# HPC-Research-Lab/GNN

Measured on AMD Instinct MI355X. Metric: mini-batches/sec + SpMM HBM GB/s, Reddit GraphSAGE/LADIES at 1/2/4/8 MI355X, higher is better.
Workload: dtype f32

## Files before the change

gnn_amd/csrc/step.hip:

```cpp
#include <hip/hip_runtime.h>
#include <rocblas/rocblas.h>

#include <algorithm>
#include <climits>
#include <cstdint>
#include <cstdlib>
#include <cstring>
#include <memory>
#include <mutex>
#include <string>

#include "common.h"
#include "gnn_layers.h"
#include "gnn_spmm.h"
#include "gnn_step.h"

namespace {

using gnn::align_up;
using gnn::ceil_div;

__global__ __launch_bounds__(256) void colsum_kernel(const float* __restrict__ dz, int M, int C,
                                                     float* __restrict__ out) {
  __shared__ float red[4];
  const int c = blockIdx.x;
  float s = 0.0f;
  for (int r = threadIdx.x; r < M; r += 256) s += dz[(int64_t)r * C + c];
#pragma unroll
  for (int m = 32; m >= 1; m >>= 1) s += __shfl_xor(s, m);
  if ((threadIdx.x & 63) == 0) red[threadIdx.x >> 6] = s;
  __syncthreads();
  if (threadIdx.x == 0) out[c] = (red[0] + red[1]) + (red[2] + red[3]);
}

struct Arena {
  char* base;
  size_t off = 0;
  template <typename T>
  T* take(int64_t count) {
    const size_t bytes = align_up((size_t)(count > 0 ? count : 1) * sizeof(T), 256);
    T* p = base ? (T*)(base + off) : nullptr;
    off += bytes;
    return p;
  }
};

int64_t L(const int64_t* d, int l, int f) { return d[GNN_STEP_HEADER + l * GNN_STEP_LAYER_SLOTS + f]; }
template <typename T>
T* P(const int64_t* d, int l, int f) {
  return (T*)(uintptr_t)L(d, l, f);
}
template <typename T>
T* HP(const int64_t* d, int f) {
  return (T*)(uintptr_t)d[f];
}

bool fills(int64_t M, int64_t N, int n) { return ceil_div(M, 128) * ceil_div(N, 128) * n >= 256; }
bool gemm_ok(const void* p, int64_t ld) { return ((uintptr_t)p % 8) == 0 && (ld % 2) == 0; }

std::mutex g_blas_mu;
rocblas_handle g_blas[64][2] = {};

int blas_handle(rocblas_handle* h, int which = 0) {
  int dev = 0;
  GNN_HIP(hipGetDevice(&dev), "hipGetDevice");
  GNN_REQUIRE(dev >= 0 && dev < 64, "gnn_train_step: device index %d", dev);
  std::lock_guard<std::mutex> g(g_blas_mu);
  if (!g_blas[dev][which]) {
    if (rocblas_create_handle(&g_blas[dev][which]) != rocblas_status_success)
      return gnn::fail(-1, "rocblas_create_handle failed");
  }
  *h = g_blas[dev][which];
  return 0;
}

struct Aux {
  hipStream_t s = nullptr;
  hipEvent_t ev[24] = {};
  int next = 0;
  std::mutex mu;
  hipEvent_t take() { return ev[next++ % 24]; }
};
std::mutex g_aux_mu;
Aux* g_aux[64][4] = {};

int aux_of(hipStream_t st, Aux** out) {
  int dev = 0;
  GNN_HIP(hipGetDevice(&dev), "hipGetDevice");
  GNN_REQUIRE(dev >= 0 && dev < 64, "gnn_train_step: device index %d", dev);
  int prio = 0, lo = 0, hi = 0;
  GNN_HIP(hipStreamGetPriority(st, &prio), "hipStreamGetPriority");
  GNN_HIP(hipDeviceGetStreamPriorityRange(&lo, &hi), "hipDeviceGetStreamPriorityRange");
  const int slot = std::min(3, std::max(0, lo - prio));
  std::lock_guard<std::mutex> g(g_aux_mu);
  Aux*& a = g_aux[dev][slot];
  if (!a) {
    std::unique_ptr<Aux> n(new Aux());
    GNN_HIP(hipStreamCreateWithPriority(&n->s, hipStreamNonBlocking, prio), "hipStreamCreateWithPriority");
    for (auto& e : n->ev) GNN_HIP(hipEventCreateWithFlags(&e, hipEventDisableTiming), "hipEventCreateWithFlags");
    a = n.release();
  }
  *out = a;
  return 0;
}

int fork_join(Aux* a, hipStream_t from, hipStream_t to) {
  hipEvent_t e = a->take();
  GNN_HIP(hipEventRecord(e, from), "hipEventRecord");
  GNN_HIP(hipStreamWaitEvent(to, e, 0), "hipStreamWaitEvent");
  return 0;
}

bool no_index() {
  const char* e = getenv("GNN_STEP_GATHER");
  const char* a = getenv("GNN_GEMM_ALGO");
  return (e && atoi(e) != 0) || (a && std::string(a) == "f32");
}

bool f32_gemm() {
  const char* e = getenv("GNN_GEMM_ALGO");
  return e && std::string(e) == "f32";
}

int gemm(int ak, int bk, int64_t M, int64_t N, int64_t K, int nb, const float* const* A, int64_t lda,
         const float* const* B, int64_t ldb, float* const* C, int64_t ldc, void* ws, size_t wsb, hipStream_t st) {
  if (f32_gemm()) return gnn_gemm_f32(ak, bk, M, N, K, nb, A, lda, B, ldb, C, ldc, ws, wsb, st);
  return gnn_gemm_f32_split3(ak, bk, M, N, K, nb, A, lda, B, ldb, C, ldc, ws, wsb, st);
}

size_t gemm_ws(int64_t M, int64_t N, int64_t K, int nb) {
  return std::max(gnn_gemm_f32_split3_workspace_bytes(M, N, K, nb), gnn_gemm_f32_workspace_bytes(M, N, K, nb));
}

bool fuse_agg_enabled() {
  const char* e = getenv("GNN_STEP_FUSE_AGG");
  return !(e && atoi(e) == 0);
}

bool small_overlap_enabled() {
  const char* e = getenv("GNN_STEP_SMALL_OVERLAP");
  return !(e && atoi(e) == 0);
}

bool overlap_enabled() {
  const char* e = getenv("GNN_STEP_OVERLAP");
  return e && atoi(e) != 0;
}

int sgemm(rocblas_handle h, rocblas_operation ta, rocblas_operation tb, int64_t m, int64_t n, int64_t k,
          const float* A, int64_t lda, const float* B, int64_t ldb, float* C, int64_t ldc) {
  const float one = 1.0f, zero = 0.0f;
  if (rocblas_sgemm(h, ta, tb, (rocblas_int)m, (rocblas_int)n, (rocblas_int)k, &one, A, (rocblas_int)lda, B,
                    (rocblas_int)ldb, &zero, C, (rocblas_int)ldc) != rocblas_status_success)
    return gnn::fail(-1, "rocblas_sgemm failed (m %lld n %lld k %lld)", (long long)m, (long long)n, (long long)k);
  return 0;
// ... 111 lines not shown
      b.b_gemm_dx = b.b_bwd = 0;
    }
  }
  for (int l = 0; l < pl.nl - 1; ++l) pl.lb[l].dY = ar.take<float>(pl.lb[l].M * pl.lb[l].D);
  return 0;
}

#define GNN_TRY(x)        \
  do {                    \
    int rc_ = (x);        \
    if (rc_) return rc_;  \
  } while (0)

}

extern "C" {

size_t gnn_train_step_workspace_bytes(const int64_t* desc) {
  if (!desc) return 0;
  Arena ar{nullptr};
  Plan pl;
  if (plan(desc, ar, pl)) return 0;
  return ar.off;
}

int gnn_train_step_f32(const int64_t* d, void* workspace, size_t workspace_bytes, void* stream) {
  GNN_REQUIRE(d != nullptr, "gnn_train_step: NULL descriptor");
  Arena ar{(char*)workspace};
  Plan pl;
  {
    Arena dry{nullptr};
    Plan tmp;
    GNN_TRY(plan(d, dry, tmp));
    GNN_REQUIRE(workspace && workspace_bytes >= dry.off, "gnn_train_step: workspace too small (%zu < %zu)",
                workspace_bytes, dry.off);
    GNN_REQUIRE((uintptr_t)workspace % 256 == 0, "gnn_train_step: workspace not 256-byte aligned");
  }
  GNN_TRY(plan(d, ar, pl));
  hipStream_t st = (hipStream_t)stream;
  rocblas_handle h = nullptr;
  GNN_TRY(blas_handle(&h));
  if (rocblas_set_stream(h, st) != rocblas_status_success) return gnn::fail(-1, "rocblas_set_stream failed");
  const int n = pl.sage ? 2 : 1;
  const float p = [&] {
    float f;
    const int32_t bits = (int32_t)d[GNN_SH_PDROP_BITS];
    std::memcpy(&f, &bits, 4);
    return f;
  }();
  const int training = (int)d[GNN_SH_TRAINING];
  Aux* aux = nullptr;
  const bool big_ov = overlap_enabled() && !f32_gemm();
  const bool small_ov = small_overlap_enabled();
  if (big_ov || small_ov) GNN_TRY(aux_of(st, &aux));
  std::unique_lock<std::mutex> aux_lock;
  if (aux) aux_lock = std::unique_lock<std::mutex>(aux->mu);
  bool aux_used = false;
  rocblas_handle ha = nullptr;
  if (aux && small_ov) {
    GNN_TRY(blas_handle(&ha, 1));
    if (rocblas_set_stream(ha, aux->s) != rocblas_status_success) return gnn::fail(-1, "rocblas_set_stream failed");
  }
  int64_t* const T = HP<int64_t>(d, GNN_SH_TIMING);
  int64_t nrec = 0;
  auto arm = [&](int64_t kind, int64_t l, int64_t M, int64_t K, int64_t nnz, int64_t F, int64_t Fk, int64_t ldx,
                 int64_t ldo, const void* X, const void* Y, int64_t res_rows) {
    if (!T || nrec >= T[0]) return;
    int64_t* r = T + 1 + GNN_STEP_TIMING_SLOTS * nrec++;
    gnn_spmm_set_timing_events((void*)r[0], (void*)r[1]);
    const int64_t v[] = {kind, l, M, K, nnz, F, Fk, ldx, ldo, (int64_t)(uintptr_t)X, (int64_t)(uintptr_t)Y, res_rows, 1};
    std::memcpy(r + 2, v, sizeof v);
  };
  auto stage_gate = [&](int l) -> int {
    if (d[GNN_SH_STAGE_EVENT] && l == (int)d[GNN_SH_STAGE_LAYER])
      GNN_HIP(hipEventRecord((hipEvent_t)d[GNN_SH_STAGE_EVENT], st), "hipEventRecord (stage gate)");
    return 0;
  };
  const int64_t phase = d[GNN_SH_PHASE];
  GNN_REQUIRE(phase >= 0 && phase <= 2, "gnn_train_step: phase %lld", (long long)phase);
  auto first_agg = [&]() -> int {
    const LayerBufs& b = pl.lb[0];
    return gnn_spmm_csr_f32(P<const int32_t>(d, 0, GNN_SL_ROWPTR), P<const int32_t>(d, 0, GNN_SL_COL),
                            P<const float>(d, 0, GNN_SL_VAL), b.M, b.K, b.nnz, b.X, b.ldx, b.feat, b.ldo, b.Fk,
                            b.ws_fwd, b.b_fwd, 0, st);
  };
  if (phase == 1) {
    GNN_TRY(first_agg());
    return stage_gate(0);
  }
  for (int l = 0; l < pl.nl; ++l) {
    LayerBufs& b = pl.lb[l];
    const int64_t N = b.N;
    const float* WB = P<const float>(d, l, GNN_SL_WB);
    const float* WW = P<const float>(d, l, GNN_SL_WW);
    if (pl.sage)
      GNN_REQUIRE(L(d, l, GNN_SL_NSAMPLED) == b.M, "gnn_train_step: layer %d sampled %lld != M %lld", l,
                  (long long)L(d, l, GNN_SL_NSAMPLED), (long long)b.M);
    const bool ok = gemm_ok(b.feat, b.ldo) && gemm_ok(WW, b.F) && (!pl.sage || gemm_ok(WB, b.F));
    const bool small_side = ha && pl.sage && !(ok && fills(b.M, N, n));
    if (big_ov && pl.sage && ok && fills(b.M, N, n)) {
      b.xs_gathered = true;
      GNN_TRY(fork_join(aux, st, aux->s));
      GNN_TRY(gnn_gather_rows_f32(b.X, b.ldx, P<const int64_t>(d, l, GNN_SL_SAMPLED), b.xs, b.ldo, nullptr, b.M, b.F,
                                  aux->s));
      const float* Ab[1] = {b.xs};
      const float* Bb[1] = {WB};
      float* Cb[1] = {b.hB};
      GNN_TRY(gnn::gemm_split3_as_batch(0, 0, b.M, N, b.F, 1, 2, 0, Ab, b.ldo, Bb, b.F, Cb, N, b.ws_gemm_f2, b.b_gemm_f,
                                        aux->s));
      if (phase != 2 || l != 0) {
        arm(0, l, b.M, b.K, b.nnz, b.F, b.Fk, b.ldx, b.ldo, b.X, b.feat, 0);
        GNN_TRY(gnn_spmm_csr_f32(P<const int32_t>(d, l, GNN_SL_ROWPTR), P<const int32_t>(d, l, GNN_SL_COL),
                                 P<const float>(d, l, GNN_SL_VAL), b.M, b.K, b.nnz, b.X, b.ldx, b.feat, b.ldo, b.Fk,
                                 b.ws_fwd, b.b_fwd, 0, st));
        GNN_TRY(stage_gate(l));
      }
      const float* Aw[1] = {b.feat};
      const float* Bw[1] = {WW};
      float* Cw[1] = {b.hW};
      GNN_TRY(gnn::gemm_split3_as_batch(0, 0, b.M, N, b.F, 1, 2, 1, Aw, b.ldo, Bw, b.F, Cw, N, b.ws_gemm_f, b.b_gemm_f, st));
      GNN_TRY(fork_join(aux, aux->s, st));
    } else if (small_side) {
      b.xs_gathered = true;
      GNN_TRY(fork_join(aux, st, aux->s));
      GNN_TRY(gnn_gather_rows_f32(b.X, b.ldx, P<const int64_t>(d, l, GNN_SL_SAMPLED), b.xs, b.ldo, nullptr, b.M,
                                  b.F, aux->s));
      GNN_TRY(mm_xwt(ha, b.xs, b.ldo, WB, b.F, b.hB, N, b.M, N, b.F));
      if (phase != 2 || l != 0) {
        arm(0, l, b.M, b.K, b.nnz, b.F, b.Fk, b.ldx, b.ldo, b.X, b.feat, 0);
        GNN_TRY(gnn_spmm_csr_f32(P<const int32_t>(d, l, GNN_SL_ROWPTR), P<const int32_t>(d, l, GNN_SL_COL),
                                 P<const float>(d, l, GNN_SL_VAL), b.M, b.K, b.nnz, b.X, b.ldx, b.feat, b.ldo, b.Fk,
                                 b.ws_fwd, b.b_fwd, 0, st));
        GNN_TRY(stage_gate(l));
      }
      GNN_TRY(mm_xwt(h, b.feat, b.ldo, WW, b.F, b.hW, N, b.M, N, b.F));
      GNN_TRY(fork_join(aux, aux->s, st));
    } else {
      if (phase != 2 || l != 0) {
        arm(0, l, b.M, b.K, b.nnz, b.F, b.Fk, b.ldx, b.ldo, b.X, b.feat, 0);
        GNN_TRY(gnn_spmm_csr_f32(P<const int32_t>(d, l, GNN_SL_ROWPTR), P<const int32_t>(d, l, GNN_SL_COL),
                                 P<const float>(d, l, GNN_SL_VAL), b.M, b.K, b.nnz, b.X, b.ldx, b.feat, b.ldo, b.Fk,
                                 b.ws_fwd, b.b_fwd, 0, st));
        GNN_TRY(stage_gate(l));
      }
      b.xs_gathered = !(pl.sage && ok && fills(b.M, N, n) && b.M >= 2048 && b.ldx == b.ldo && !no_index());
      if (pl.sage && b.xs_gathered)
        GNN_TRY(gnn_gather_rows_f32(b.X, b.ldx, P<const int64_t>(d, l, GNN_SL_SAMPLED), b.xs, b.ldo, nullptr, b.M,
                                    b.F, st));
    }
    if ((big_ov && pl.sage && ok && fills(b.M, N, n)) || small_side) {
    } else if (ok && fills(b.M, N, n) && !b.xs_gathered) {
      const float* A[2] = {b.X, b.feat};
      const int64_t* IA[2] = {P<const int64_t>(d, l, GNN_SL_SAMPLED), nullptr};
      const float* B[2] = {WB, WW};
      float* Cc[2] = {b.hB, b.hW};
      GNN_TRY(gnn::gemm_split3_indexed(0, 0, b.M, N, b.F, n, A, b.ldo, IA, b.K, B, b.F, nullptr, 0, Cc, N,
                                       b.ws_gemm_f, b.b_gemm_f, st));
    } else if (ok && fills(b.M, N, n)) {
      const float* A[2] = {pl.sage ? b.xs : b.feat, b.feat};
      const float* B[2] = {pl.sage ? WB : WW, WW};
      float* Cc[2] = {pl.sage ? b.hB : b.hW, b.hW};
      GNN_TRY(gemm(0, 0, b.M, N, b.F, n, A + (pl.sage ? 0 : 1), b.ldo, B + (pl.sage ? 0 : 1), b.F,
                                  Cc + (pl.sage ? 0 : 1), N, b.ws_gemm_f, b.b_gemm_f, st));
    } else {
      if (pl.sage) GNN_TRY(mm_xwt(h, b.xs, b.ldo, WB, b.F, b.hB, N, b.M, N, b.F));
      GNN_TRY(mm_xwt(h, b.feat, b.ldo, WW, b.F, b.hW, N, b.M, N, b.F));
    }
    GNN_TRY(gnn_sage_norm_fwd_f32(pl.sage ? b.hB : nullptr, pl.sage ? N : 4, pl.sage ? N : 0, b.hW, N, N,
                                  pl.sage ? P<const float>(d, l, GNN_SL_BB) : nullptr, P<const float>(d, l, GNN_SL_BW),
                                  P<const float>(d, l, GNN_SL_SCALE), P<const float>(d, l, GNN_SL_OFFSET), b.M, p,
                                  (uint64_t)L(d, l, GNN_SL_SEED), training, b.Y, b.D, b.mean, b.rstd, st));
  }
  const LayerBufs& top = pl.lb[pl.nl - 1];
  const float* Wh = HP<const float>(d, GNN_SH_HEAD_W);
  const uint64_t hseed = (uint64_t)d[GNN_SH_HEAD_SEED];
  const float* labels = HP<const float>(d, GNN_SH_LABELS);
  const int64_t ldl = d[GNN_SH_LDL];
  GNN_TRY(gnn_head_bce_fwd_f32(top.Y, top.D, pl.Mh, pl.Dh, Wh, HP<const float>(d, GNN_SH_HEAD_B), pl.C, labels, ldl, p,
                               hseed, training, pl.xd, pl.z, pl.nrm, pl.rowloss, HP<float>(d, GNN_SH_LOSS), st));
  GNN_TRY(gnn_head_bce_bwd_f32(top.Y, top.D, pl.Mh, pl.Dh, Wh, pl.C, labels, ldl, nullptr, p, hseed, training, pl.z,
                               pl.nrm, pl.dz, pl.dXh, pl.Dh, st));
  const int64_t* const E = HP<const int64_t>(d, GNN_SH_GRAD_EVENTS);
  auto grads_ready = [&](int64_t slot, hipStream_t s) -> int {
    if (E && slot < E[0] && E[slot]) GNN_HIP(hipEventRecord((hipEvent_t)E[slot], s), "hipEventRecord (grad event)");
    return 0;
  };
  bool head_pending = true;
  auto head_grads = [&](hipStream_t s, rocblas_handle hh) -> int {
    GNN_TRY(mm_gtx(hh, pl.dz, pl.C, pl.xd, pl.Dh, HP<float>(d, GNN_SH_HEAD_GW), pl.Dh, pl.C, pl.Dh, pl.Mh));
    if (HP<float>(d, GNN_SH_HEAD_GB)) {
// ... 116 lines not shown
```

gnn_amd/executor.py:

```python
from __future__ import annotations

import os
import struct
from typing import List, Optional

import numpy as np
import torch

from . import _lib
from . import custom_sparse_ops as cso

VERSION, MAX_LAYERS, HEADER, LAYER_SLOTS, SAGE, GCN = 1, 4, 24, 32, 0, 1
(H_VERSION, H_LAYERS, H_KIND, H_X0, H_LDX0, H_F0, H_HEAD_W, H_HEAD_B, H_HEAD_GW, H_HEAD_GB, H_CLASSES, H_LABELS,
 H_LDL, H_HEAD_SEED, H_PDROP_BITS, H_TRAINING, H_LOSS, H_NHID, H_TIMING, H_GRAD_EVENTS, H_STAGE_EVENT,
 H_STAGE_LAYER, H_PHASE) = range(23)
TIMING_SLOTS = 16
(L_ROWPTR, L_COL, L_VAL, L_M, L_K, L_NNZ, L_TROWPTR, L_TCOL, L_TVAL, L_SAMPLED, L_NSAMPLED, L_RMAP, L_WW, L_BW,
 L_WB, L_BB, L_SCALE, L_OFFSET, L_GWW, L_GBW, L_GWB, L_GBB, L_GSCALE, L_GOFFSET, L_SEED) = range(25)


def _p(t: Optional[torch.Tensor]) -> int:
    return 0 if t is None else t.data_ptr()


def enabled() -> bool:
    return os.environ.get("GNN_NATIVE_STEP", "1") != "0"


class NativeStep:

    def __init__(self, model):
        from . import models

        enc = model.encoder
        if not getattr(enc, "fused", False):
            raise ValueError("NativeStep needs the fused model (build_model(..., fused=True))")
        if isinstance(enc, models.GraphSage):
            self.kind = SAGE
        elif isinstance(enc, models.GCN):
            self.kind = GCN
        else:
            raise ValueError(f"NativeStep: unsupported encoder {type(enc).__name__}")
        if any(g.order != 1 for g in enc.gcs) or not 1 <= len(enc.gcs) <= MAX_LAYERS:
            raise ValueError("NativeStep: every layer must have order 1 (1-4 layers)")
        self.model = model
        self.enc = enc
        self.params: List[torch.nn.Parameter] = [p for p in model.parameters()]
        dev = self.params[0].device
        self.device = dev
        n = sum(p.numel() for p in self.params)
        self.flat_grad = torch.zeros(n, dtype=torch.float32, device=dev)
        self.grads, off = [], 0
        for p in self.params:
            self.grads.append(self.flat_grad[off:off + p.numel()].view_as(p))
            off += p.numel()
        g = {id(p): gr for p, gr in zip(self.params, self.grads)}
        d = np.zeros(HEADER + LAYER_SLOTS * len(enc.gcs), dtype=np.int64)
        d[H_VERSION] = VERSION
        d[H_LAYERS] = len(enc.gcs)
        d[H_KIND] = self.kind
        head = model.linear
        d[H_HEAD_W], d[H_HEAD_B] = _p(head.weight), _p(head.bias)
        d[H_HEAD_GW], d[H_HEAD_GB] = _p(g[id(head.weight)]), _p(g.get(id(head.bias)) if head.bias is not None else None)
        d[H_CLASSES] = head.weight.shape[0]
        d[H_NHID] = enc.gcs[0].n_out
        self.p_enc = float(enc.dropout.p)
        self.p_head = float(model.dropout.p)
        if self.p_enc != self.p_head:
# ... 10 lines not shown
            d[b + L_WW], d[b + L_BW] = _p(W.weight), _p(W.bias)
            d[b + L_GWW], d[b + L_GBW] = _p(g[id(W.weight)]), _p(g[id(W.bias)])
            d[b + L_SCALE], d[b + L_OFFSET] = _p(gc.scale), _p(gc.offset)
            d[b + L_GSCALE], d[b + L_GOFFSET] = _p(g[id(gc.scale)]), _p(g[id(gc.offset)])
        for p in self.params:
            if not (p.is_cuda and p.dtype == torch.float32 and p.is_contiguous()):
                raise ValueError("NativeStep: parameters must be contiguous float32 CUDA tensors")
        self.template = d

    def supports(self, x0, adjs, sampled_nodes, labels) -> bool:
        from .custom_sparse_ops import CsrOperand

        if not (x0.is_cuda and x0.dtype == torch.float32 and x0.stride(1) == 1 and labels.dtype == torch.float32
                and labels.dim() == 2 and labels.stride(1) == 1):
            return False
        C, D = self.model.linear.weight.shape
        if C > 256 or D % 4 or D > 2048 or labels.shape[1] != C:
            return False
        for li, op in enumerate(adjs):
            if not isinstance(op, CsrOperand):
                return False
            if li >= 1 and op._t is None:
                return False
            if self.kind == SAGE:
                s = sampled_nodes[li]
                if s.dtype != torch.int64 or not s.is_contiguous() or s.numel() != op.shape[0]:
                    return False
                if li >= 1 and getattr(s, "_gnn_rmap", None) is None:
                    return False
        return True

    def grad_stages(self):
        head = {id(p) for p in self.model.linear.parameters()}
        stages = [[i for i, p in enumerate(self.params) if id(p) in head]]
        for gc in reversed(self.enc.gcs):
            mine = {id(p) for p in gc.parameters()}
            stages.append([i for i, p in enumerate(self.params) if id(p) in mine])
        return stages

    @staticmethod
    def _batch_key(x0, adjs, labels):
        return (x0.data_ptr(), tuple(x0.shape), x0.stride(0), labels.data_ptr(), tuple(id(op) for op in adjs))

    def prefetch(self, x0, adjs, sampled_nodes, labels, stage_gate=None) -> None:
        d = self._desc(x0, adjs, sampled_nodes, labels, seeds=False)
        if stage_gate is not None and int(stage_gate[1]) == 0:
            self._set_gate(d, stage_gate)
        d[H_PHASE] = 1
        ws, wsb = self._workspace(d, x0.device)
        L = _lib.lib()
        with _lib.on_device(x0.device):
            _lib.check(L.gnn_train_step_f32(d.ctypes.data, ws.data_ptr(), wsb, _lib.stream_of(x0.device)),
                       "gnn_train_step_f32 (phase 1)")
        self._pre = (self._batch_key(x0, adjs, labels), ws, wsb, (x0, tuple(adjs), labels))

    def drop_prefetch(self) -> None:
        self._pre = None

    @staticmethod
    def _set_gate(d, stage_gate):
        ev, layer = stage_gate
        if not getattr(ev, "_gnn_created", False):
            ev.record()
            ev._gnn_created = True
        d[H_STAGE_EVENT], d[H_STAGE_LAYER] = ev.cuda_event, int(layer)

    @staticmethod
    def _workspace(d, device):
        wsb = _lib.lib().gnn_train_step_workspace_bytes(d.ctypes.data)
        if wsb == 0:
            raise RuntimeError("gnn_train_step_workspace_bytes: " + _lib.lib().gnn_last_error().decode(errors="replace"))
        return torch.empty(wsb, dtype=torch.uint8, device=device), wsb

    def step(self, x0, adjs, sampled_nodes, labels, grad_events=None, stage_gate=None) -> torch.Tensor:
        d = self._desc(x0, adjs, sampled_nodes, labels, seeds=True)
        pre, self._pre = getattr(self, "_pre", None), None
        if pre is not None and pre[0] == self._batch_key(x0, adjs, labels):
            d[H_PHASE] = 2
            ws, wsb = pre[1], pre[2]
            if stage_gate is not None and int(stage_gate[1]) == 0:
                stage_gate = None
        else:
            ws, wsb = None, 0
        loss = torch.empty((), dtype=torch.float32, device=x0.device)
        d[H_LOSS] = loss.data_ptr()
        timing = self._arm_timing(d, len(adjs)) if cso.timing_enabled() else None
        E = None
        if grad_events is not None:
            E = np.zeros(1 + len(grad_events), dtype=np.int64)
            E[0] = len(E)
            for i, ev in enumerate(grad_events):
                if ev is not None:
                    ev.record()
                    E[1 + i] = ev.cuda_event
            d[H_GRAD_EVENTS] = E.ctypes.data
        if stage_gate is not None:
            self._set_gate(d, stage_gate)
        L = _lib.lib()
        dp = d.ctypes.data
        if ws is None:
            ws, wsb = self._workspace(d, x0.device)
        with _lib.on_device(x0.device):
            _lib.check(L.gnn_train_step_f32(dp, ws.data_ptr(), wsb, _lib.stream_of(x0.device)), "gnn_train_step_f32")
        if timing is not None:
            self._collect_timing(*timing)
        for p, gr in zip(self.params, self.grads):
            p.grad = gr
        return loss

    def _desc(self, x0, adjs, sampled_nodes, labels, seeds: bool):
        model = self.model
        training = model.training
        tr = bool(training and self.p_enc > 0)
        d = self.template.copy()
        d[H_X0], d[H_LDX0], d[H_F0] = x0.data_ptr(), x0.stride(0) if x0.shape[0] > 1 else x0.shape[1], x0.shape[1]
        d[H_LABELS], d[H_LDL] = labels.data_ptr(), labels.stride(0) if labels.shape[0] > 1 else labels.shape[1]
        d[H_TRAINING] = int(tr)
        sv = torch.randint(0, 2**62, (len(adjs) + 1,)).tolist() if (tr and seeds) else None
        for li, op in enumerate(adjs):
            b = HEADER + li * LAYER_SLOTS
            d[b + L_ROWPTR], d[b + L_COL], d[b + L_VAL] = op.rowptr.data_ptr(), op.col.data_ptr(), op.val.data_ptr()
            d[b + L_M], d[b + L_K], d[b + L_NNZ] = op.shape[0], op.shape[1], op.nnz
            if li >= 1:
                t = op._t
                d[b + L_TROWPTR], d[b + L_TCOL], d[b + L_TVAL] = t.rowptr.data_ptr(), t.col.data_ptr(), t.val.data_ptr()
            if self.kind == SAGE:
                s = sampled_nodes[li]
                d[b + L_SAMPLED], d[b + L_NSAMPLED] = s.data_ptr(), s.numel()
                r = getattr(s, "_gnn_rmap", None)
                d[b + L_RMAP] = _p(r) if li >= 1 else 0
            d[b + L_SEED] = sv[li] if sv is not None else 0
        d[H_HEAD_SEED] = sv[len(adjs)] if sv is not None else 0
        return d

    @staticmethod
    def _arm_timing(d, nl):
        n = 2 * nl - 1
        T = np.zeros(1 + TIMING_SLOTS * n, dtype=np.int64)
        T[0] = n
        evs = []
        for i in range(n):
            e0, e1 = torch.cuda.Event(enable_timing=True), torch.cuda.Event(enable_timing=True)
            e0.record()
            e1.record()
            T[1 + TIMING_SLOTS * i], T[2 + TIMING_SLOTS * i] = e0.cuda_event, e1.cuda_event
            evs.append((e0, e1))
        d[H_TIMING] = T.ctypes.data
        return T, evs

    @staticmethod
    def _collect_timing(T, evs):
        for i, (e0, e1) in enumerate(evs):
            r = T[1 + TIMING_SLOTS * i: 1 + TIMING_SLOTS * (i + 1)]
            if r[14] != 1:
                continue
            kind, l, M, K, nnz, F, Fk, ldx, ldy, xp, yp, res = (int(v) for v in r[2:14])
# ... 3 lines not shown
```

gnn_amd/staging.py:

```python
from __future__ import annotations

import contextlib
import ctypes
import os
import sys
import weakref
from dataclasses import dataclass
from typing import List, Optional

import numpy as np
import torch

from . import custom_sparse_ops as cso


_WAIT_SLEEP_S = max(0.0, float(os.environ.get("GNN_WAIT_SLEEP_US", "20")) * 1e-6)
_slack_set = set()


def wait_event(ev) -> None:
    if _WAIT_SLEEP_S <= 0.0:
        ev.synchronize()
        return
    if ev.query():
# ... 68 lines not shown


@dataclass
class StagePlan:
    n_input: int
    own_pos: np.ndarray
    own_src: np.ndarray
    host_pos: np.ndarray
    host_rows: Optional[torch.Tensor]
    peer_pos: List[np.ndarray]
    peer_src: List[np.ndarray]
    pinned: tuple = ()
    blob: object = None
    peer_meta: object = None


def make_plan(host_batch, store: FeatureStore, rank: int, world_size: int, devices=None) -> StagePlan:
    devices = list(range(world_size)) if devices is None else list(devices)
    masks = host_batch.input_nodes_mask_on_devices
    idxs = host_batch.nodes_idx_on_devices
    own_pos = np.flatnonzero(masks[rank]).astype(np.int64)
    own_src = np.asarray(idxs[rank], dtype=np.int64)
    host_pos = np.flatnonzero(host_batch.input_nodes_mask_on_cpu).astype(np.int64)
    host_src = np.ascontiguousarray(host_batch.nodes_idx_on_cpu, dtype=np.int64)
    host_rows = None if store.zero_copy else store.host_rows_pinned(host_src)
    peer_pos, peer_src = [], []
    for j in range(world_size):
        if j == rank:
            peer_pos.append(np.zeros(0, np.int64))
            peer_src.append(np.zeros(0, np.int64))
        else:
            peer_pos.append(np.flatnonzero(masks[j]).astype(np.int64))
            peer_src.append(np.asarray(idxs[j], dtype=np.int64))
    cuda = torch.cuda.is_available()
    arrs = (own_pos, own_src, host_pos) + ((host_src,) if store.zero_copy else ())
    pin = tuple(torch.from_numpy(a).pin_memory() if cuda else torch.from_numpy(a) for a in arrs)
    return StagePlan(host_batch.num_input_nodes, own_pos, own_src, host_pos, host_rows, peer_pos, peer_src, pin)


def _staging_stream(device):
    cus = int(os.environ.get("GNN_STAGE_CUS", "0"))
    if cus <= 0:
        return torch.cuda.Stream(device=device)
    import ctypes

    from . import _lib

    ptr = ctypes.c_void_p()
    idx = torch.device(device).index or 0
    _lib.check(_lib.lib().gnn_stream_create_cu_masked(idx, cus, 0, ctypes.byref(ptr)), "gnn_stream_create_cu_masked")
    return torch.cuda.ExternalStream(ptr.value, device=device)


class Stager:

    def __init__(self, store: FeatureStore, exchange: Optional["PeerExchange"] = None):
        self.store = store
        self.device = store.device
        self.stream = _staging_stream(self.device)
        self.exchange = exchange
        self.timing: Optional[list] = None
        self.gate: Optional[torch.cuda.Event] = None

    def take_timing(self):
        recs, self.timing = self.timing or [], None
        if not recs:
            return 0, 0.0
        recs[-1][1].synchronize()
        return sum(b for _, _, b in recs), sum(a.elapsed_time(b) for a, b, _ in recs) * 1e-3

    def issue(self, plan: StagePlan, batch_fn=None):
        dev = self.device
        st = self.stream
        meta = None
        if self.exchange is not None:
            fut = plan.peer_meta
            if fut is not None:
                plan.peer_meta = None
                meta = fut.result()
            else:
                meta = self.exchange.prepare(plan)
        with torch.cuda.stream(st):
            x0 = torch.empty((plan.n_input, self.store.ld), dtype=torch.float32, device=dev)
            if _NATIVE_STAGE and plan.blob is not None and self.timing is None and not self.store.zero_copy:
                from .loader import ToDevice

                if isinstance(batch_fn, ToDevice) and batch_fn.host is plan.blob:
                    batch = plan.blob.stage(dev, x0, self.store, self.gate)
                    if batch_fn.on_built is not None:
                        batch_fn.on_built(batch)
                    extra = self.exchange.exchange(plan, x0, self.store, meta) if self.exchange is not None else ()
                    ev = torch.cuda.Event()
                    ev.record(st)
                    return StagedX0(x0, ev, tuple(extra) + tuple(batch.tensors()), self.store.F, batch)
            nh = len(plan.host_pos)
            if self.timing is not None:
                e0, e1 = torch.cuda.Event(enable_timing=True), torch.cuda.Event(enable_timing=True)
                e0.record(st)
            if plan.blob is not None:
                own_pos, own_src, host_pos, host_dev = plan.blob.stage_views(dev)
                if self.store.zero_copy:
                    cso.gather_rows_host(self.store.host, host_dev, x0, host_pos, n=nh)
            else:
                idx = [t.to(dev, non_blocking=True) for t in plan.pinned]
                own_pos, own_src, host_pos = idx[:3]
                if plan.host_rows is None:
                    host_dev = idx[3]
                    cso.gather_rows_host(self.store.host, host_dev, x0, host_pos, n=nh)
                else:
                    host_dev = plan.host_rows.to(dev, non_blocking=True)
            if self.timing is not None:
                e1.record(st)
                self.timing.append((e0, e1, plan.blob.nbytes if plan.blob is not None else nh * self.store.ld * 4))
            if self.gate is not None:
                st.wait_event(self.gate)
            host_rows_here = nh and (plan.host_rows is not None or (plan.blob is not None and not self.store.zero_copy))
            if host_rows_here and _GATHER2:
                cso.gather_rows2(self.store.gpu_buffer, own_src, own_pos, len(plan.own_pos), host_dev, None, host_pos,
                                 nh, x0)
            else:
                cso.gather_rows(self.store.gpu_buffer, own_src, x0, own_pos, n=len(plan.own_pos))
                if host_rows_here:
                    cso.gather_rows(host_dev, None, x0, host_pos, n=nh)
            extra = ()
            if self.exchange is not None:
                extra = self.exchange.exchange(plan, x0, self.store, meta)
            batch = batch_fn() if batch_fn is not None else None
            ev = torch.cuda.Event()
            ev.record(st)
        keep = (own_pos, own_src, host_pos, host_dev) + tuple(extra)
        if batch is not None:
            keep += tuple(batch.tensors())
        return StagedX0(x0, ev, keep, self.store.F, batch)


_EXTRACT_CHECK = os.environ.get("GNN_EXTRACT_CHECK", "step")
_GATHER2 = os.environ.get("GNN_GATHER2", "1") != "0"
_NATIVE_STAGE = os.environ.get("GNN_NATIVE_STAGE", "1") != "0" and _GATHER2


class StagedX0:
    def __init__(self, x0, event, keep, F, batch=None):
        self._x0 = x0
        self.event = event
        self._keep = keep
        self.F = F
        self.batch = batch
        self.adjs = list(batch.adjs) if batch is not None and batch.adjs is not None else None
        self.err_host = getattr(batch, "err_host", None) if batch is not None else None

    def wait(self, retire: Optional["Retirement"] = None) -> torch.Tensor:
        b = self.batch
        if b is not None and self.err_host is not None and _EXTRACT_CHECK == "step":
            wait_event(self.event)
            b.check_extraction(self.err_host)
        cur = torch.cuda.current_stream(self._x0.device)
        cur.wait_event(self.event)
        if retire is None:
            self._x0.record_stream(cur)
            for t in self._keep:
                t.record_stream(cur)
        return self._x0[:, : self.F]


class Retirement:

    def __init__(self, depth: int = 3):
        import collections

        self.depth = depth
        self.q = collections.deque()
        self.wait_s = 0.0

    def retire(self, staged) -> None:
        ev = torch.cuda.Event()
        ev.record()
        self.q.append((ev, staged))
        while self.q and self.q[0][0].query():
            self.q.popleft()
        if len(self.q) > self.depth:
            import time

            t0 = time.perf_counter()
            while len(self.q) > self.depth:
                ev0, _ = self.q.popleft()
                wait_event(ev0)
            self.wait_s += time.perf_counter() - t0

    def drain(self) -> None:
        while self.q:
            ev0, _ = self.q.popleft()
            ev0.synchronize()


class NegotiatedStream:

    def __init__(self, it, exchange: "PeerExchange", depth: int = 4):
        import collections
        from concurrent.futures import ThreadPoolExecutor

        self.it = iter(it)
        self.exchange = exchange
        self.depth = max(0, int(depth))
        self.q = collections.deque()
# ... 217 lines not shown
```

gnn_amd/train.py:

```python
from __future__ import annotations

import os
from typing import Optional

import torch
from torch._utils import _flatten_dense_tensors, _unflatten_dense_tensors

from .models import loss as loss_fn


class Trainer:
    def __init__(self, model: torch.nn.Module, lr: float, device, group=None, sigmoid_loss: bool = True,
                 clip: float = 5.0):
        self.model = model
        self.device = torch.device(device)
        self.sigmoid_loss = sigmoid_loss
        self.clip = clip
        self.group = group
        self.params = [p for p in model.parameters() if p.requires_grad]
        self.native = self.device.type == "cuda"
        if self.native:
            torch.backends.cuda.preferred_blas_library("cublas")
            from .optim import ClipAdam

# ... 26 lines not shown
        self.exchange = self.bucketed if os.environ.get("GNN_DP_BUCKETS", "0") == "1" else None
        self.stage_gate = None

    @property
    def num_params(self) -> int:
        return sum(p.numel() for p in self.params)

    def broadcast_parameters(self):
        flat = _flatten_dense_tensors([p.detach() for p in self.params])
        torch.distributed.broadcast(flat, src=0, group=self.group)
        with torch.no_grad():
            for p, v in zip(self.params, _unflatten_dense_tensors(flat, self.params)):
                p.copy_(v)

    def param_digest(self) -> str:
        import hashlib

        h = hashlib.sha256()
        for p in self.params:
            h.update(p.detach().contiguous().cpu().numpy().tobytes())
        return h.hexdigest()[:16]

    def check_ranks_agree(self) -> dict:
        d = self.param_digest()
        dist = torch.distributed
        if not (dist.is_available() and dist.is_initialized()):
            return {"identical": True, "digests": [d]}
        digests = [None] * dist.get_world_size(self.group)
        torch.distributed.all_gather_object(digests, d, group=self.group)
        return {"identical": all(x == digests[0] for x in digests), "digests": digests}

    def allreduce_grads(self) -> Optional[torch.Tensor]:
        if not self.dp:
            return None
        grads = [p.grad for p in self.params]
        flat = _flatten_dense_tensors(grads)
        torch.distributed.all_reduce(flat, op=torch.distributed.ReduceOp.SUM, group=self.group)
        for p, g in zip(self.params, _unflatten_dense_tensors(flat, grads)):
            p.grad = g
        return flat

    def _next_batch(self, prefetch):
        if prefetch is None or self.executor is None or os.environ.get("GNN_PREFETCH_L0", "1") == "0":
            return None
        from . import custom_sparse_ops as cso

        if cso.timing_enabled():
            return None
        nxt = prefetch() if callable(prefetch) else prefetch
        if nxt is None or not self.executor.supports(*nxt):
            return None
        return nxt

    def step(self, x0, adjs, sampled_nodes, labels, prefetch=None) -> torch.Tensor:
        if not self.model.training:
            self.model.train()
        if self.executor is not None and self.executor.supports(x0, adjs, sampled_nodes, labels):
            if self.exchange is not None:
                loss = self.executor.step(x0, adjs, sampled_nodes, labels, grad_events=self.exchange.events,
                                          stage_gate=self.stage_gate)
                self.exchange.issue()
                self.exchange.finish()
                self.optimizer.step(clipped=True)
                return loss
            loss = self.executor.step(x0, adjs, sampled_nodes, labels,
                                      stage_gate=self.stage_gate)
            if self.dp:
                flat = self.optimizer.clip_to_flat()
                work = torch.distributed.all_reduce(flat, op=torch.distributed.ReduceOp.SUM, group=self.group,
                                                    async_op=True)
                nxt = self._next_batch(prefetch)
                if nxt is not None:
                    self.executor.prefetch(*nxt, stage_gate=self.stage_gate)
                work.wait()
                self.optimizer.step(clipped=True)
            else:
                self.optimizer.step()
            return loss
        for p in self.params:
            p.grad = None
        if hasattr(self.model, "forward_loss"):
            loss, _ = self.model.forward_loss(x0, adjs, sampled_nodes, labels, self.sigmoid_loss)
        else:
            out = self.model(x0, adjs, sampled_nodes)
            loss = loss_fn(out, labels, self.sigmoid_loss, self.device)
        if self.native:
            one = getattr(self, "_one", None)
            if one is None or one.device != loss.device:
                one = self._one = torch.ones((), dtype=loss.dtype, device=loss.device)
            loss.backward(one)
        else:
            loss.backward()
        if self.native:
            if self.dp:
                flat = self.optimizer.clip_to_flat()
                torch.distributed.all_reduce(flat, op=torch.distributed.ReduceOp.SUM, group=self.group)
                self.optimizer.step(clipped=True)
            else:
                self.optimizer.step()
            return loss.detach()
        torch.nn.utils.clip_grad_norm_(self.params, self.clip)
        self.allreduce_grads()
        self.optimizer.step()
        return loss.detach()


DEFAULT_TIMEOUT_S = 180.0


def collective_timeout():
    import datetime

    s = float(os.environ.get("GNN_DIST_TIMEOUT_S", DEFAULT_TIMEOUT_S))
    if not s > 0:
        raise ValueError(f"GNN_DIST_TIMEOUT_S must be > 0, got {s}")
    return datetime.timedelta(seconds=s)


def init_group(backend: str, rank: Optional[int] = None, world: Optional[int] = None, local: int = 0):
# ... 34 lines not shown
```

include/gnn_step.h:

```cpp
#ifndef GNN_STEP_H
#define GNN_STEP_H

#include <stddef.h>
#include <stdint.h>

#ifdef __cplusplus
extern "C" {
#endif

#define GNN_STEP_VERSION 1
#define GNN_STEP_MAX_LAYERS 4
#define GNN_STEP_HEADER 24
#define GNN_STEP_LAYER_SLOTS 32
#define GNN_STEP_SAGE 0
#define GNN_STEP_GCN 1
#define GNN_STEP_TIMING_SLOTS 16

enum {
  GNN_SH_VERSION = 0, GNN_SH_LAYERS = 1, GNN_SH_KIND = 2, GNN_SH_X0 = 3, GNN_SH_LDX0 = 4, GNN_SH_F0 = 5,
  GNN_SH_HEAD_W = 6, GNN_SH_HEAD_B = 7, GNN_SH_HEAD_GW = 8, GNN_SH_HEAD_GB = 9, GNN_SH_CLASSES = 10,
  GNN_SH_LABELS = 11, GNN_SH_LDL = 12, GNN_SH_HEAD_SEED = 13, GNN_SH_PDROP_BITS = 14, GNN_SH_TRAINING = 15,
  GNN_SH_LOSS = 16, GNN_SH_NHID = 17, GNN_SH_TIMING = 18, GNN_SH_GRAD_EVENTS = 19, GNN_SH_STAGE_EVENT = 20,
  GNN_SH_STAGE_LAYER = 21, GNN_SH_PHASE = 22
};
enum {
  GNN_SL_ROWPTR = 0, GNN_SL_COL = 1, GNN_SL_VAL = 2, GNN_SL_M = 3, GNN_SL_K = 4, GNN_SL_NNZ = 5,
  GNN_SL_TROWPTR = 6, GNN_SL_TCOL = 7, GNN_SL_TVAL = 8, GNN_SL_SAMPLED = 9, GNN_SL_NSAMPLED = 10,
  GNN_SL_RMAP = 11, GNN_SL_WW = 12, GNN_SL_BW = 13, GNN_SL_WB = 14, GNN_SL_BB = 15, GNN_SL_SCALE = 16,
  GNN_SL_OFFSET = 17, GNN_SL_GWW = 18, GNN_SL_GBW = 19, GNN_SL_GWB = 20, GNN_SL_GBB = 21, GNN_SL_GSCALE = 22,
  GNN_SL_GOFFSET = 23, GNN_SL_SEED = 24
};

size_t gnn_train_step_workspace_bytes(const int64_t* desc);
int gnn_train_step_f32(const int64_t* desc, void* workspace, size_t workspace_bytes, void* stream);

#ifdef __cplusplus
}
#endif

#endif
```

Baseline: 608.0.

## Overlap next batch's first-layer SpMM with current step on a prefetch stream

Inside a training step, the first-layer aggregation SpMM of the next staged mini-batch is now issued on a separate low-priority prefetch stream, forked when the current step reaches its last layer. The goal is to hide that SpMM behind the tail and backward pass of the current step. A staging FIFO exposes the next staged batch, and the executor keeps the prefetched workspace and a done event so the next step can skip phase 1. This brings cross-step event plumbing, an extra workspace allocation per step, and contention for HBM bandwidth between the two streams. It is turned off for data-parallel runs, when timing is enabled, and when the stage gate sits at layer 0.

```diff
diff --git a/gnn_amd/csrc/step.hip b/gnn_amd/csrc/step.hip
--- a/gnn_amd/csrc/step.hip
+++ b/gnn_amd/csrc/step.hip
@@ -76,6 +76,7 @@
 
 struct Aux {
   hipStream_t s = nullptr;
+  hipStream_t pf = nullptr;
   hipEvent_t ev[24] = {};
   int next = 0;
   std::mutex mu;
@@ -101,6 +102,16 @@
     a = n.release();
   }
   *out = a;
+  return 0;
+}
+
+int prefetch_stream(Aux* a, hipStream_t* out) {
+  if (!a->pf) {
+    int lo = 0, hi = 0;
+    GNN_HIP(hipDeviceGetStreamPriorityRange(&lo, &hi), "hipDeviceGetStreamPriorityRange");
+    GNN_HIP(hipStreamCreateWithPriority(&a->pf, hipStreamNonBlocking, lo), "hipStreamCreateWithPriority");
+  }
+  *out = a->pf;
   return 0;
 }
 
@@ -318,7 +329,8 @@
   Aux* aux = nullptr;
   const bool big_ov = overlap_enabled() && !f32_gemm();
   const bool small_ov = small_overlap_enabled();
-  if (big_ov || small_ov) GNN_TRY(aux_of(st, &aux));
+  const int64_t* const NX = HP<const int64_t>(d, GNN_SH_NEXT);
+  if (big_ov || small_ov || NX) GNN_TRY(aux_of(st, &aux));
   std::unique_lock<std::mutex> aux_lock;
   if (aux) aux_lock = std::unique_lock<std::mutex>(aux->mu);
   bool aux_used = false;
@@ -344,14 +356,52 @@
   };
   const int64_t phase = d[GNN_SH_PHASE];
   GNN_REQUIRE(phase >= 0 && phase <= 2, "gnn_train_step: phase %lld", (long long)phase);
-  auto first_agg = [&]() -> int {
-    const LayerBufs& b = pl.lb[0];
-    return gnn_spmm_csr_f32(P<const int32_t>(d, 0, GNN_SL_ROWPTR), P<const int32_t>(d, 0, GNN_SL_COL),
-                            P<const float>(d, 0, GNN_SL_VAL), b.M, b.K, b.nnz, b.X, b.ldx, b.feat, b.ldo, b.Fk,
-                            b.ws_fwd, b.b_fwd, 0, st);
+  auto first_agg = [](const int64_t* dd, const Plan& pp, hipStream_t s) -> int {
+    const LayerBufs& b = pp.lb[0];
+    return gnn_spmm_csr_f32(P<const int32_t>(dd, 0, GNN_SL_ROWPTR), P<const int32_t>(dd, 0, GNN_SL_COL),
+                            P<const float>(dd, 0, GNN_SL_VAL), b.M, b.K, b.nnz, b.X, b.ldx, b.feat, b.ldo, b.Fk,
+                            b.ws_fwd, b.b_fwd, 0, s);
+  };
+  const int64_t* nd = nullptr;
+  Plan npl;
+  hipStream_t ps = nullptr;
+  if (NX) {
+    GNN_REQUIRE(phase != 1, "gnn_train_step: a next batch with phase 1");
+    GNN_REQUIRE(!(d[GNN_SH_STAGE_EVENT] && d[GNN_SH_STAGE_LAYER] == 0),
+                "gnn_train_step: a next batch with the staging gate at layer 0");
+    nd = HP<const int64_t>(NX, GNN_SN_DESC);
+    void* const nws = HP<void>(NX, GNN_SN_WORKSPACE);
+    const size_t nwsb = (size_t)NX[GNN_SN_WORKSPACE_BYTES];
+    GNN_REQUIRE(nd != nullptr && NX[GNN_SN_DONE] != 0, "gnn_train_step: next batch without descriptor or done event");
+    GNN_REQUIRE(nd[GNN_SH_NEXT] == 0 && nd[GNN_SH_TIMING] == 0, "gnn_train_step: next batch's descriptor is not plain");
+    Arena dry{nullptr};
+    Plan tmp;
+    GNN_TRY(plan(nd, dry, tmp));
+    GNN_REQUIRE(nws && nwsb >= dry.off, "gnn_train_step: next batch's workspace too small (%zu < %zu)", nwsb, dry.off);
+    GNN_REQUIRE((uintptr_t)nws % 256 == 0, "gnn_train_step: next batch's workspace not 256-byte aligned");
+    Arena nar{(char*)nws};
+    GNN_TRY(plan(nd, nar, npl));
+    ps = (hipStream_t)NX[GNN_SN_STREAM];
+    if (!ps) GNN_TRY(prefetch_stream(aux, &ps));
+  }
+  auto issue_next = [&](hipEvent_t e) -> int {
+    GNN_HIP(hipStreamWaitEvent(ps, e, 0), "hipStreamWaitEvent (prefetch fork)");
+    if (NX[GNN_SN_READY])
+      GNN_HIP(hipStreamWaitEvent(ps, (hipEvent_t)NX[GNN_SN_READY], 0), "hipStreamWaitEvent (prefetch ready)");
+    GNN_TRY(first_agg(nd, npl, ps));
+    GNN_HIP(hipEventRecord((hipEvent_t)NX[GNN_SN_DONE], ps), "hipEventRecord (prefetch done)");
+    return 0;
+  };
+  auto fork_fwd = [&](int l, bool to_aux) -> int {
+    if (!to_aux && !(NX && l == pl.nl - 1)) return 0;
+    hipEvent_t e = aux->take();
+    GNN_HIP(hipEventRecord(e, st), "hipEventRecord");
+    if (to_aux) GNN_HIP(hipStreamWaitEvent(aux->s, e, 0), "hipStreamWaitEvent");
+    if (NX && l == pl.nl - 1) GNN_TRY(issue_next(e));
+    return 0;
   };
   if (phase == 1) {
-    GNN_TRY(first_agg());
+    GNN_TRY(first_agg(d, pl, st));
     return stage_gate(0);
   }
   for (int l = 0; l < pl.nl; ++l) {
@@ -366,7 +416,7 @@
     const bool small_side = ha && pl.sage && !(ok && fills(b.M, N, n));
     if (big_ov && pl.sage && ok && fills(b.M, N, n)) {
       b.xs_gathered = true;
-      GNN_TRY(fork_join(aux, st, aux->s));
+      GNN_TRY(fork_fwd(l, true));
       GNN_TRY(gnn_gather_rows_f32(b.X, b.ldx, P<const int64_t>(d, l, GNN_SL_SAMPLED), b.xs, b.ldo, nullptr, b.M, b.F,
                                   aux->s));
       const float* Ab[1] = {b.xs};
@@ -388,7 +438,7 @@
       GNN_TRY(fork_join(aux, aux->s, st));
     } else if (small_side) {
       b.xs_gathered = true;
-      GNN_TRY(fork_join(aux, st, aux->s));
+      GNN_TRY(fork_fwd(l, true));
       GNN_TRY(gnn_gather_rows_f32(b.X, b.ldx, P<const int64_t>(d, l, GNN_SL_SAMPLED), b.xs, b.ldo, nullptr, b.M,
                                   b.F, aux->s));
       GNN_TRY(mm_xwt(ha, b.xs, b.ldo, WB, b.F, b.hB, N, b.M, N, b.F));
@@ -402,6 +452,7 @@
       GNN_TRY(mm_xwt(h, b.feat, b.ldo, WW, b.F, b.hW, N, b.M, N, b.F));
       GNN_TRY(fork_join(aux, aux->s, st));
     } else {
+      GNN_TRY(fork_fwd(l, false));
       if (phase != 2 || l != 0) {
         arm(0, l, b.M, b.K, b.nnz, b.F, b.Fk, b.ldx, b.ldo, b.X, b.feat, 0);
         GNN_TRY(gnn_spmm_csr_f32(P<const int32_t>(d, l, GNN_SL_ROWPTR), P<const int32_t>(d, l, GNN_SL_COL),
diff --git a/gnn_amd/executor.py b/gnn_amd/executor.py
--- a/gnn_amd/executor.py
+++ b/gnn_amd/executor.py
@@ -13,7 +13,8 @@
 VERSION, MAX_LAYERS, HEADER, LAYER_SLOTS, SAGE, GCN = 1, 4, 24, 32, 0, 1
 (H_VERSION, H_LAYERS, H_KIND, H_X0, H_LDX0, H_F0, H_HEAD_W, H_HEAD_B, H_HEAD_GW, H_HEAD_GB, H_CLASSES, H_LABELS,
  H_LDL, H_HEAD_SEED, H_PDROP_BITS, H_TRAINING, H_LOSS, H_NHID, H_TIMING, H_GRAD_EVENTS, H_STAGE_EVENT,
- H_STAGE_LAYER, H_PHASE) = range(23)
+ H_STAGE_LAYER, H_PHASE, H_NEXT) = range(24)
+(N_DESC, N_WORKSPACE, N_WORKSPACE_BYTES, N_READY, N_DONE, N_STREAM) = range(6)
 TIMING_SLOTS = 16
 (L_ROWPTR, L_COL, L_VAL, L_M, L_K, L_NNZ, L_TROWPTR, L_TCOL, L_TVAL, L_SAMPLED, L_NSAMPLED, L_RMAP, L_WW, L_BW,
  L_WB, L_BB, L_SCALE, L_OFFSET, L_GWW, L_GBW, L_GWB, L_GBB, L_GSCALE, L_GOFFSET, L_SEED) = range(25)
@@ -130,10 +131,36 @@
         with _lib.on_device(x0.device):
             _lib.check(L.gnn_train_step_f32(d.ctypes.data, ws.data_ptr(), wsb, _lib.stream_of(x0.device)),
                        "gnn_train_step_f32 (phase 1)")
-        self._pre = (self._batch_key(x0, adjs, labels), ws, wsb, (x0, tuple(adjs), labels))
+        self._release(getattr(self, "_pre", None))
+        self._pre = (self._batch_key(x0, adjs, labels), ws, wsb, (x0, tuple(adjs), labels), None, ())
 
     def drop_prefetch(self) -> None:
-        self._pre = None
+        pre, self._pre = getattr(self, "_pre", None), None
+        self._release(pre)
+
+    @staticmethod
+    def _release(pre) -> None:
+        if pre is None or pre[4] is None:
+            return
+        for st in pre[5]:
+            if st is not None:
+                st.wait_event(pre[4])
+
+    def __del__(self):
+        try:
+            self.drop_prefetch()
+        except Exception:
+            pass
+
+    def _done_event(self):
+        ring = getattr(self, "_done_ring", None)
+        if ring is None:
+            ring = self._done_ring = [torch.cuda.Event() for _ in range(4)]
+            for ev in ring:
+                ev.record()
+            self._done_i = 0
+        self._done_i = (self._done_i + 1) % len(ring)
+        return ring[self._done_i]
 
     @staticmethod
     def _set_gate(d, stage_gate):
@@ -150,16 +177,23 @@
             raise RuntimeError("gnn_train_step_workspace_bytes: " + _lib.lib().gnn_last_error().decode(errors="replace"))
         return torch.empty(wsb, dtype=torch.uint8, device=device), wsb
 
-    def step(self, x0, adjs, sampled_nodes, labels, grad_events=None, stage_gate=None) -> torch.Tensor:
+    def step(self, x0, adjs, sampled_nodes, labels, grad_events=None, stage_gate=None, next=None) -> torch.Tensor:
         d = self._desc(x0, adjs, sampled_nodes, labels, seeds=True)
         pre, self._pre = getattr(self, "_pre", None), None
+        cur = torch.cuda.current_stream(x0.device)
         if pre is not None and pre[0] == self._batch_key(x0, adjs, labels):
             d[H_PHASE] = 2
             ws, wsb = pre[1], pre[2]
+            if pre[4] is not None:
+                cur.wait_event(pre[4])
             if stage_gate is not None and int(stage_gate[1]) == 0:
                 stage_gate = None
         else:
+            self._release(pre)
             ws, wsb = None, 0
+        del pre
+        if next is not None and (cso.timing_enabled() or (stage_gate is not None and int(stage_gate[1]) == 0)):
+            next = None
         loss = torch.empty((), dtype=torch.float32, device=x0.device)
         d[H_LOSS] = loss.data_ptr()
         timing = self._arm_timing(d, len(adjs)) if cso.timing_enabled() else None
@@ -178,8 +212,24 @@
         dp = d.ctypes.data
         if ws is None:
             ws, wsb = self._workspace(d, x0.device)
+        pending = None
+        if next is not None:
+            (nx0, nadjs, nsampled, nlabels), ready, nstream = next
+            on_staging = nstream is not None and os.environ.get("GNN_PREFETCH_STREAM", "staging") != "own"
+            dn = self._desc(nx0, nadjs, nsampled, nlabels, seeds=False)
+            nws, nwsb = self._workspace(dn, x0.device)
+            done = self._done_event()
+            R = np.zeros(6, dtype=np.int64)
+            R[N_DESC], R[N_WORKSPACE], R[N_WORKSPACE_BYTES] = dn.ctypes.data, nws.data_ptr(), nwsb
+            R[N_READY] = ready.cuda_event if ready is not None else 0
+            R[N_DONE] = done.cuda_event
+            R[N_STREAM] = nstream.cuda_stream if on_staging else 0
+            d[H_NEXT] = R.ctypes.data
+            pending = (self._batch_key(nx0, nadjs, nlabels), nws, nwsb, (nx0, tuple(nadjs), nlabels), done,
+                       (cur, nstream))
         with _lib.on_device(x0.device):
             _lib.check(L.gnn_train_step_f32(dp, ws.data_ptr(), wsb, _lib.stream_of(x0.device)), "gnn_train_step_f32")
+        self._pre = pending
         if timing is not None:
             self._collect_timing(*timing)
         for p, gr in zip(self.params, self.grads):
diff --git a/gnn_amd/staging.py b/gnn_amd/staging.py
--- a/gnn_amd/staging.py
+++ b/gnn_amd/staging.py
@@ -144,6 +144,48 @@
     return torch.cuda.ExternalStream(ptr.value, device=device)
 
 
+class StageFifo:
+
+    def __init__(self):
+        self._q = {}
+
+    @staticmethod
+    def _key(device):
+        d = torch.device(device)
+        return (d.type, d.index or 0)
+
+    def push(self, device, item) -> None:
+        import collections
+
+        q = self._q.setdefault(self._key(device), collections.deque())
+        while q and q[0]() is None:
+            q.popleft()
+        q.append(weakref.ref(item))
+
+    def remove(self, device, item) -> None:
+        q = self._q.get(self._key(device))
+        if not q:
+            return
+        for r in list(q):
+            if r() is item or r() is None:
+                q.remove(r)
+
+    def head(self, device):
+        q = self._q.get(self._key(device))
+        while q:
+            item = q[0]()
+            if item is not None:
+                return item
+            q.popleft()
+        return None
+
+    def __len__(self):
+        return sum(1 for q in self._q.values() for r in q if r() is not None)
+
+
+STAGED = StageFifo()
+
+
 class Stager:
 
     def __init__(self, store: FeatureStore, exchange: Optional["PeerExchange"] = None):
@@ -184,7 +226,7 @@
                     extra = self.exchange.exchange(plan, x0, self.store, meta) if self.exchange is not None else ()
                     ev = torch.cuda.Event()
                     ev.record(st)
-                    return StagedX0(x0, ev, tuple(extra) + tuple(batch.tensors()), self.store.F, batch)
+                    return self._staged(StagedX0(x0, ev, tuple(extra) + tuple(batch.tensors()), self.store.F, batch))
             nh = len(plan.host_pos)
             if self.timing is not None:
                 e0, e1 = torch.cuda.Event(enable_timing=True), torch.cuda.Event(enable_timing=True)
@@ -223,7 +265,12 @@
         keep = (own_pos, own_src, host_pos, host_dev) + tuple(extra)
         if batch is not None:
             keep += tuple(batch.tensors())
-        return StagedX0(x0, ev, keep, self.store.F, batch)
+        return self._staged(StagedX0(x0, ev, keep, self.store.F, batch))
+
+    def _staged(self, staged):
+        staged.stream = self.stream
+        STAGED.push(self.device, staged)
+        return staged
 
 
 _EXTRACT_CHECK = os.environ.get("GNN_EXTRACT_CHECK", "step")
@@ -240,8 +287,16 @@
         self.batch = batch
         self.adjs = list(batch.adjs) if batch is not None and batch.adjs is not None else None
         self.err_host = getattr(batch, "err_host", None) if batch is not None else None
+        self.stream = None
+
+    def peek(self):
+        b = self.batch
+        if b is None or self.adjs is None:
+            return None
+        return self._x0[:, : self.F], self.adjs, b.sampled_nodes, b.labels
 
     def wait(self, retire: Optional["Retirement"] = None) -> torch.Tensor:
+        STAGED.remove(self._x0.device, self)
         b = self.batch
         if b is not None and self.err_host is not None and _EXTRACT_CHECK == "step":
             wait_event(self.event)
diff --git a/gnn_amd/train.py b/gnn_amd/train.py
--- a/gnn_amd/train.py
+++ b/gnn_amd/train.py
@@ -102,6 +102,20 @@
             return None
         return nxt
 
+    def _staged_next(self, prefetch):
+        if prefetch is not None or os.environ.get("GNN_PREFETCH_L0", "1") == "0":
+            return None
+        from . import custom_sparse_ops as cso
+        from .staging import STAGED
+
+        if cso.timing_enabled():
+            return None
+        head = STAGED.head(self.device)
+        nxt = head.peek() if head is not None else None
+        if nxt is None or not self.executor.supports(*nxt):
+            return None
+        return nxt, head.event, head.stream
+
     def step(self, x0, adjs, sampled_nodes, labels, prefetch=None) -> torch.Tensor:
         if not self.model.training:
             self.model.train()
@@ -114,7 +128,8 @@
                 self.optimizer.step(clipped=True)
                 return loss
             loss = self.executor.step(x0, adjs, sampled_nodes, labels,
-                                      stage_gate=self.stage_gate)
+                                      stage_gate=self.stage_gate,
+                                      next=None if self.dp else self._staged_next(prefetch))
             if self.dp:
                 flat = self.optimizer.clip_to_flat()
                 work = torch.distributed.all_reduce(flat, op=torch.distributed.ReduceOp.SUM, group=self.group,
diff --git a/include/gnn_step.h b/include/gnn_step.h
--- a/include/gnn_step.h
+++ b/include/gnn_step.h
@@ -21,7 +21,12 @@
   GNN_SH_HEAD_W = 6, GNN_SH_HEAD_B = 7, GNN_SH_HEAD_GW = 8, GNN_SH_HEAD_GB = 9, GNN_SH_CLASSES = 10,
   GNN_SH_LABELS = 11, GNN_SH_LDL = 12, GNN_SH_HEAD_SEED = 13, GNN_SH_PDROP_BITS = 14, GNN_SH_TRAINING = 15,
   GNN_SH_LOSS = 16, GNN_SH_NHID = 17, GNN_SH_TIMING = 18, GNN_SH_GRAD_EVENTS = 19, GNN_SH_STAGE_EVENT = 20,
-  GNN_SH_STAGE_LAYER = 21, GNN_SH_PHASE = 22
+  GNN_SH_STAGE_LAYER = 21, GNN_SH_PHASE = 22, GNN_SH_NEXT = 23
+};
+#define GNN_STEP_NEXT_SLOTS 6
+enum {
+  GNN_SN_DESC = 0, GNN_SN_WORKSPACE = 1, GNN_SN_WORKSPACE_BYTES = 2, GNN_SN_READY = 3, GNN_SN_DONE = 4,
+  GNN_SN_STREAM = 5
 };
 enum {
   GNN_SL_ROWPTR = 0, GNN_SL_COL = 1, GNN_SL_VAL = 2, GNN_SL_M = 3, GNN_SL_K = 4, GNN_SL_NNZ = 5,
```

After: 619.6, median of 6. +1.9%, better.
